# qingqing-zijin/LEAD-YOLO

Measured on AMD Instinct MI355X. Metric: images/sec (640x640) fwd+bwd, higher is better.
Workload: dtype bf16; 1 GPU; lead-yolo-s bs=64/gpu 3x640x640 bf16 full train step: uint8 batch -> train-mode forward (batch-statistics BN), ComputeLoss, HIP backward, clip 10, SGD-nesterov 3 groups, ModelEMA update (BASELINE.json configs[2]); random-init weights; global_batch=64, parallelism=dp1 (single GPU, no collective), world_size=1

## Files before the change

### lead-yolo_amd/csrc/ly_conv3x3.hip

```cpp
#include <cstdlib>
#include "ly_tile.hpp"
#include "ly_params.h"

#define LY_C3_NT 8
#define LY_C3_NV 6

#ifndef LY_C3_NTA_WPE
#define LY_C3_NTA_WPE 3
#endif
template <typename T, int MT, int WC, int NTA = 0>
__global__ __launch_bounds__(LY_THREADS) __attribute__((amdgpu_waves_per_eu(sizeof(T) == 2 ? (NTA > 0 ? LY_C3_NTA_WPE : 3) : 2))) void ly_conv3x3_kernel(const LyConv3Params P, const int gy, const int tiles_x, const int tiles_y, const int rp, const int ps) {
  using TR = LyT<T>;
  using RV = typename TR::RV;
  constexpr int VW = TR::VW, PL = TR::PL;
  constexpr int LY_CC = 8 * VW;
  constexpr int KS = LY_CC / 32;
  constexpr int LY_RSH = ly_qrs(KS);
  extern __shared__ f32x4 ly_smem4[];
  const int TH = P.TH, TW = P.TW, FW = TW + 2;
  const int frame = (TH + 2) * FW;
  char* hs_hi = reinterpret_cast<char*>(ly_smem4);
  char* hs_lo = hs_hi + (PL - 1) * 4 * ps;
  const T* const x = reinterpret_cast<const T*>(P.x);
  T* const out = reinterpret_cast<T*>(P.out);

  const int tid = threadIdx.x, lane = tid & 63;
  const int wave = __builtin_amdgcn_readfirstlane(tid >> 6);
  const int li = lane & 15, lq = lane >> 4;
  constexpr int WP = 4 / WC;
  constexpr int NTW = LY_C3_NT / WP;
  const int wc = wave % WC, wp = wave / WC;
  int b = ly_xcd_remap((int)blockIdx.x, (int)gridDim.x);
  const int by = b % gy; b /= gy;
  const int tx = b % tiles_x; b /= tiles_x;
  const int ty = b % tiles_y;
  const int n_img = b / tiles_y;
  const int h0 = ty * TH, w0 = tx * TW;
  const int npx = TH * TW;
  const int ntv = (npx + 15) >> 4;
  const f32x4 zero = ly_zero4();
  const int C32 = (P.Cin + 31) >> 5;
  const int NCH = (P.Cin + LY_CC - 1) / LY_CC;
  const int S = 9 * C32;
  const int Tt = (P.N + 15) >> 4;
  const long img0 = (long)n_img * P.H * P.W;

  int hb[NTW];
  long orow[NTW];
#pragma unroll
  for (int n = 0; n < NTW; ++n) {
    const int p = 16 * (wp * NTW + n) + li;
    const int pp = p < npx ? p : 0;
    const int r = pp / TW, c = pp - r * TW;
    hb[n] = r * rp + c * LY_RSH;
    const bool ok = p < npx && h0 + r < P.H && w0 + c < P.W;
    orow[n] = ok ? img0 + (long)(h0 + r) * P.W + (w0 + c) : -1;
  }

  const int items = frame * 8;
  int src[LY_C3_NV];
  int dst[LY_C3_NV];
#pragma unroll
  for (int e = 0; e < LY_C3_NV; ++e) {
    const int idx = tid + e * LY_THREADS;
    int off = -1;
    int dd = 0;
    if (idx < items) {
      const int pos = idx >> 3, c4 = idx & 7;
      const int fr = pos / FW, fc = pos - fr * FW;
      const int hh = h0 - 1 + fr, ww = w0 - 1 + fc;
      dd = fr * rp + fc * LY_RSH;
      if (hh >= 0 && hh < P.H && ww >= 0 && ww < P.W) off = (int)((img0 + (long)hh * P.W + ww) * P.ldx + VW * c4);
    }
    src[e] = off; dst[e] = dd;
  }
  RV pv[LY_C3_NV];
  auto prefetch = [&](int c0) {
#pragma unroll
    for (int e = 0; e < LY_C3_NV; ++e) {
      const int c4 = (tid + e * LY_THREADS) & 7;
      const bool ok = src[e] >= 0 && c0 + VW * c4 < P.Cin;
      pv[e] = ly_ldrv<T>(ok ? x + src[e] + c0 : x);
    }
  };
  auto commit = [&](int c0) {
#pragma unroll
    for (int e = 0; e < LY_C3_NV; ++e) {
      const int idx = tid + e * LY_THREADS;
      const int c4 = idx & 7;
      const bool ok = src[e] >= 0 && c0 + VW * c4 < P.Cin;
      RV v = pv[e];
      if (!ok) ly_zero_raw(v);
      if (idx < items) ly_img_put_rv(hs_hi, hs_lo, dst[e], ps, VW * c4, v);
    }
  };

  f32x4 acc[MT][NTW];
#pragma unroll
  for (int t = 0; t < MT; ++t)
#pragma unroll
    for (int n = 0; n < NTW; ++n) acc[t][n] = zero;
  long wbase[MT];
#pragma unroll
  for (int t = 0; t < MT; ++t) {
    const int tt = (by * WC + wc) * MT + t;
    wbase[t] = (long)(tt < Tt ? tt : Tt - 1) * S;
  }
  const uint4* wpk = reinterpret_cast<const uint4*>(P.wp);
  ly_l2_warm(P.wp, (long)Tt * S * PL * 1024, P.stats ? reinterpret_cast<float*>(P.stats) : reinterpret_cast<float*>(P.out));

  auto wstep = [&](int tap, int cc, int ks) -> long {
    int st = KS * cc + ks;
    if (st >= C32) st = C32 - 1;
    return (long)tap * C32 + st;
  };
  LyWF<PL> wcur[MT], wnxt[MT];
#pragma unroll
  for (int t = 0; t < MT; ++t) wcur[t] = ly_wfragp<PL>(wpk, wbase[t], lane);

  prefetch(0);
  commit(0);
  __syncthreads();

  for (int cc = 0; cc < NCH; ++cc) {
    const bool more = cc + 1 < NCH;
    prefetch((more ? cc + 1 : cc) * LY_CC);
#pragma unroll(MT * NTW <= 8 ? 1 : 9)
    for (int tap = 0; tap < 9; ++tap) {
      const int toff = (tap / 3) * rp + (tap % 3) * LY_RSH;
#pragma unroll
      for (int ks = 0; ks < KS; ++ks) {
        {
          const bool last = ks == KS - 1;
          const int nk = last ? 0 : ks + 1;
          const int nt = last ? (tap < 8 ? tap + 1 : 0) : tap;
          const int nc = (last && tap == 8) ? (more ? cc + 1 : cc) : cc;
#pragma unroll
          for (int t = 0; t < MT; ++t) wnxt[t] = ly_wfragp<PL>(wpk, wbase[t] + wstep(nt, nc, nk), lane);
        }
        if constexpr (NTA > 0) {
          bf16x8 xh[NTA], xl[NTA];
#pragma unroll
          for (int n = 0; n < NTA; ++n) {
            xh[n] = ly_img_frag(hs_hi, hb[n] + toff, ps, ks, lq);
            xl[n] = xh[n];
            if constexpr (PL == 2) xl[n] = ly_img_frag(hs_lo, hb[n] + toff, ps, ks, lq);
          }
#pragma unroll
          for (int n = 0; n < NTA; ++n)
#pragma unroll
            for (int t = 0; t < MT; ++t) acc[t][n] = ly_mfmap<PL>(wcur[t], xh[n], xl[n], acc[t][n]);
        } else {
#pragma unroll
        for (int n = 0; n < NTW; ++n) {
          if (wp * NTW + n < ntv) {
            const bf16x8 xh = ly_img_frag(hs_hi, hb[n] + toff, ps, ks, lq);
            bf16x8 xl = xh;
            if constexpr (PL == 2) xl = ly_img_frag(hs_lo, hb[n] + toff, ps, ks, lq);
#pragma unroll
            for (int t = 0; t < MT; ++t) acc[t][n] = ly_mfmap<PL>(wcur[t], xh, xl, acc[t][n]);
          }
        }
        }
#pragma unroll
        for (int t = 0; t < MT; ++t) wcur[t] = wnxt[t];
      }
    }
    if (more) {
      __syncthreads();
      commit((cc + 1) * LY_CC);
      __syncthreads();
    }
  }

  const int act = P.act;
  const bool vec_ok = (P.ldo & 3) == 0;
#pragma unroll
  for (int t = 0; t < MT; ++t) {
    const int tt = (by * WC + wc) * MT + t;
    const int c = 16 * tt + 4 * lq;
    if (tt >= Tt || c >= P.N) continue;
    float sc[4], sh[4];
#pragma unroll
    for (int r = 0; r < 4; ++r) {
      const bool ok = c + r < P.N;
      sc[r] = (ok && P.e_scale) ? P.e_scale[c + r] : 1.f;
      sh[r] = (ok && P.e_shift) ? P.e_shift[c + r] : 0.f;
    }
    f32x4 s1 = zero, s2 = zero;
#pragma unroll
    for (int n = 0; n < NTW; ++n) {
      if (orow[n] < 0) continue;
      f32x4 u;
#pragma unroll
      for (int r = 0; r < 4; ++r) u[r] = acc[t][n][r] * sc[r] + sh[r];
      if (P.stats) {
        s1 += u;
        s2 += u * u;
        if (!out) continue;
      }
      const f32x4 v = ly_act4(u, act);
      T* o = out + orow[n] * P.ldo + c;
      if (vec_ok && c + 3 < P.N) {
        ly_st4<T>(o, v);
      } else {
#pragma unroll
        for (int r = 0; r < 4; ++r)
          if (c + r < P.N) ly_st1<T>(o + r, v[r]);
      }
    }
    if (P.stats) ly_stats_flush(P.stats, P.N, c, s1, s2);
  }
}

#ifndef LY_C3_PD
#define LY_C3_PD 3
#endif
template <int V>
struct LyC3Ic { static constexpr int value = V; };

template <typename T, int MT, int WC>
__global__ __launch_bounds__(LY_THREADS) __attribute__((amdgpu_waves_per_eu(2))) void ly_conv3x3_lat_kernel(const LyConv3Params P, const int gy, const int tiles_x, const int tiles_y, const int rp, const int ps) {
  using TR = LyT<T>;
  using RV = typename TR::RV;
  constexpr int VW = TR::VW, PL = TR::PL;
  constexpr int LY_CC = 8 * VW;
  constexpr int KS = LY_CC / 32;
  constexpr int LY_RSH = ly_qrs(KS);
  extern __shared__ f32x4 ly_smem4[];
  const int TH = P.TH, TW = P.TW, FW = TW + 2;
  const int frame = (TH + 2) * FW;
  char* hs_hi = reinterpret_cast<char*>(ly_smem4);
  char* hs_lo = hs_hi + (PL - 1) * 4 * ps;
  const T* const x = reinterpret_cast<const T*>(P.x);
  T* const out = reinterpret_cast<T*>(P.out);

  const int tid = threadIdx.x, lane = tid & 63;
  const int wave = __builtin_amdgcn_readfirstlane(tid >> 6);
  const int li = lane & 15, lq = lane >> 4;
  constexpr int WP = 4 / WC;
  constexpr int NTW = LY_C3_NT / WP;
  const int wc = wave % WC, wp = wave / WC;
  int b = ly_xcd_remap((int)blockIdx.x, (int)gridDim.x);
  const int by = b % gy; b /= gy;
  const int tx = b % tiles_x; b /= tiles_x;
  const int ty = b % tiles_y;
  const int n_img = b / tiles_y;
  const int h0 = ty * TH, w0 = tx * TW;
  const int npx = TH * TW;
  const int ntv = (npx + 15) >> 4;
  const f32x4 zero = ly_zero4();
  const int C32 = (P.Cin + 31) >> 5;
  const int NCH = (P.Cin + LY_CC - 1) / LY_CC;
  const int S = 9 * C32;
  const int Tt = (P.N + 15) >> 4;
  const long img0 = (long)n_img * P.H * P.W;

  int hb[NTW];
#pragma unroll
  for (int n = 0; n < NTW; ++n) {
    const int p = 16 * (wp * NTW + n) + li;
    const int pp = p < npx ? p : 0;
    const int r = pp / TW, c = pp - r * TW;
    hb[n] = r * rp + c * LY_RSH;
  }
  auto out_row = [&](int n) -> long {
    const int p = 16 * (wp * NTW + n) + li;
    const int pp = p < npx ? p : 0;
    const int r = pp / TW, c = pp - r * TW;
    const bool ok = p < npx && h0 + r < P.H && w0 + c < P.W;
    return ok ? img0 + (long)(h0 + r) * P.W + (w0 + c) : -1;
  };

  const int items = frame * 8;
  int src[LY_C3_NV];
  int dst[LY_C3_NV];
#pragma unroll
  for (int e = 0; e < LY_C3_NV; ++e) {
    const int idx = tid + e * LY_THREADS;
    int off = -1;
    int dd = 0;
    if (idx < items) {
      const int pos = idx >> 3, c4 = idx & 7;
      const int fr = pos / FW, fc = pos - fr * FW;
      const int hh = h0 - 1 + fr, ww = w0 - 1 + fc;
      dd = fr * rp + fc * LY_RSH;
      if (hh >= 0 && hh < P.H && ww >= 0 && ww < P.W) off = (int)((img0 + (long)hh * P.W + ww) * P.ldx + VW * c4);
    }
    src[e] = off; dst[e] = dd;
  }
  RV pv[LY_C3_NV];
  auto prefetch = [&](int c0) {
#pragma unroll
    for (int e = 0; e < LY_C3_NV; ++e) {
      const int c4 = (tid + e * LY_THREADS) & 7;
      const bool ok = src[e] >= 0 && c0 + VW * c4 < P.Cin;
      pv[e] = ly_ldrv<T>(ok ? x + src[e] + c0 : x);
    }
  };
  auto commit = [&](int c0) {
#pragma unroll
    for (int e = 0; e < LY_C3_NV; ++e) {
      const int idx = tid + e * LY_THREADS;
      const int c4 = idx & 7;
      const bool ok = src[e] >= 0 && c0 + VW * c4 < P.Cin;
      RV v = pv[e];
      if (!ok) ly_zero_raw(v);
      if (idx < items) ly_img_put_rv(hs_hi, hs_lo, dst[e], ps, VW * c4, v);
    }
  };

  f32x4 acc[MT][NTW];
#pragma unroll
  for (int t = 0; t < MT; ++t)
#pragma unroll
    for (int n = 0; n < NTW; ++n) acc[t][n] = zero;
  long wbase[MT];
#pragma unroll
  for (int t = 0; t < MT; ++t) {
    const int tt = (by * WC + wc) * MT + t;
    wbase[t] = (long)(tt < Tt ? tt : Tt - 1) * S;
  }
  const uint4* wpk = reinterpret_cast<const uint4*>(P.wp);
  ly_l2_warm(P.wp, (long)Tt * S * PL * 1024, P.stats ? reinterpret_cast<float*>(P.stats) : reinterpret_cast<float*>(P.out));

  auto wstep = [&](int tap, int cc, int ks) -> long {
    int st = KS * cc + ks;
    if (st >= C32) st = C32 - 1;
    return (long)tap * C32 + st;
  };
  static_assert(PL == 1, "bf16 storage only");
  constexpr int PD = LY_C3_PD;
  constexpr int SPC = 9 * KS;
  static_assert(SPC % PD == 0, "ring depth must divide the steps of a chunk");
  LyWF<PL> wq[PD][MT];
  auto wstep_at = [&](int cc, int j, bool more) -> long {
    int c2 = cc;
    if (j >= SPC) { j -= SPC; c2 = more ? cc + 1 : cc; }
    return wstep(j / KS, c2, j % KS);
  };
  {
#pragma unroll
    for (int j = 0; j < PD - 1; ++j)
#pragma unroll
      for (int t = 0; t < MT; ++t) wq[j][t] = ly_wfragp<PL>(wpk, wbase[t] + wstep_at(0, j, NCH > 1), lane);
  }

  prefetch(0);
  commit(0);
  __syncthreads();

  auto contract = [&](auto ncC) {
    constexpr int NC = decltype(ncC)::value;
    for (int cc = 0; cc < NCH; ++cc) {
      const bool more = cc + 1 < NCH;
      prefetch((more ? cc + 1 : cc) * LY_CC);
      {
#pragma unroll
        for (int tap = 0; tap < 9; ++tap) {
          int toff = (tap / 3) * rp + (tap % 3) * LY_RSH;
          asm volatile("" : "+s"(toff));
#pragma unroll
          for (int ks = 0; ks < KS; ++ks) {
            const int j = tap * KS + ks;
            int lane_j = lane;
            asm volatile("" : "+v"(lane_j));
#pragma unroll
            for (int t = 0; t < MT; ++t) wq[(j + PD - 1) % PD][t] = ly_wfragp<PL>(wpk, wbase[t] + wstep_at(cc, j + PD - 1, more), lane_j);
#pragma unroll
            for (int n = 0; n < NC; ++n) {
              {
                const bf16x8 xh = ly_img_frag(hs_hi, hb[n] + toff, ps, ks, lq);
#pragma unroll
                for (int t = 0; t < MT; ++t) acc[t][n] = ly_mfmap<PL>(wq[j % PD][t], xh, xh, acc[t][n]);
              }
            }
            __builtin_amdgcn_sched_barrier(0);
          }
        }
      }
      if (more) {
        __syncthreads();
        commit((cc + 1) * LY_CC);
        __syncthreads();
      }
    }
  };
  {
    int nw = ntv - wp * NTW;
    nw = nw < 0 ? 0 : nw > NTW ? NTW : nw;
    switch (nw) {
      case 1: contract(LyC3Ic<1>()); break;
      case 2: contract(LyC3Ic<2>()); break;
      case 3: contract(LyC3Ic<3>()); break;
      case 4: contract(LyC3Ic<(NTW >= 4 ? 4 : NTW)>()); break;
      case 5: contract(LyC3Ic<(NTW >= 5 ? 5 : NTW)>()); break;
      case 6: contract(LyC3Ic<(NTW >= 6 ? 6 : NTW)>()); break;
      case 7: contract(LyC3Ic<(NTW >= 7 ? 7 : NTW)>()); break;
      case 8: contract(LyC3Ic<(NTW >= 8 ? 8 : NTW)>()); break;
      default: contract(LyC3Ic<0>()); break;
    }
  }

  const int act = P.act;
  const bool vec_ok = (P.ldo & 3) == 0;
#pragma unroll
  for (int t = 0; t < MT; ++t) {
    const int tt = (by * WC + wc) * MT + t;
    const int c = 16 * tt + 4 * lq;
    if (tt >= Tt || c >= P.N) continue;
    float sc[4], sh[4];
#pragma unroll
    for (int r = 0; r < 4; ++r) {
      const bool ok = c + r < P.N;
      sc[r] = (ok && P.e_scale) ? P.e_scale[c + r] : 1.f;
      sh[r] = (ok && P.e_shift) ? P.e_shift[c + r] : 0.f;
    }
    f32x4 s1 = zero, s2 = zero;
#pragma unroll
    for (int n = 0; n < NTW; ++n) {
      const long orow_n = out_row(n);
      if (orow_n < 0) continue;
      f32x4 u;
#pragma unroll
      for (int r = 0; r < 4; ++r) u[r] = acc[t][n][r] * sc[r] + sh[r];
      if (P.stats) {
        s1 += u;
        s2 += u * u;
        if (!out) continue;
      }
      const f32x4 v = ly_act4(u, act);
      T* o = out + orow_n * P.ldo + c;
      if (vec_ok && c + 3 < P.N) {
        ly_st4<T>(o, v);
      } else {
#pragma unroll
        for (int r = 0; r < 4; ++r)
          if (c + r < P.N) ly_st1<T>(o + r, v[r]);
      }
    }
    if (P.stats) ly_stats_flush(P.stats, P.N, c, s1, s2);
  }
}

static int conv3_row_pitch(int TH, int TW, int rsh) {
  const int FW = TW + 2, npx = TH * TW;
  int best = FW * rsh, best_w = 1 << 30;
  for (int rp = FW * rsh; rp < FW * rsh + 256; rp += 16) {
    int worst = 0;
    for (int n = 0; 16 * n < npx; ++n) {
      int cnt[16] = {0};
      for (int li = 0; li < 16; ++li) {
        const int p = 16 * n + li, pp = p < npx ? p : 0;
        const int c = ++cnt[(((pp / TW) * rp + (pp % TW) * rsh) >> 4) & 15];
        if (p < npx && c > worst) worst = c;
      }
    }
    if (worst < best_w) { best_w = worst; best = rp; }
    if (worst <= 1) break;
  }
  return best;
}

template <typename T, int MT, int WC, bool LAT = false, int NTA = 0>
static int launch_conv3(const LyConv3Params& P, const LyOut& out) {
  const int tiles_x = (P.W + P.TW - 1) / P.TW, tiles_y = (P.H + P.TH - 1) / P.TH;
  const int gy = (P.N + 16 * MT * WC - 1) / (16 * MT * WC);
  const long n_img = P.M / ((long)P.H * P.W);
  long nb = n_img * tiles_x * tiles_y * gy;
  LY_CHECK(nb < (1L << 31), "conv3x3: grid too large");
  const int rp = conv3_row_pitch(P.TH, P.TW, ly_qrs(8 * LyT<T>::VW / 32));
  const int ps = ly_qps((P.TH + 2) * rp);
  size_t lds = LyT<T>::PL * (size_t)4 * ps;
  if constexpr (LAT)
    return LY_EMIT(out, (ly_launch_lds<ly_conv3x3_lat_kernel<T, MT, WC>>(dim3((unsigned)nb), dim3(LY_THREADS), lds, out.st, P, gy, tiles_x, tiles_y, rp, ps)),
                   "ly_conv3x3_lat_kernel<%s, %d, %d>", ly_tname<T>(), MT, WC);
  else
    return LY_EMIT(out, (ly_launch_lds<ly_conv3x3_kernel<T, MT, WC, NTA>>(dim3((unsigned)nb), dim3(LY_THREADS), lds, out.st, P, gy, tiles_x, tiles_y, rp, ps)),
                   "ly_conv3x3_kernel<%s, %d, %d, %d>", ly_tname<T>(), MT, WC, NTA);
}

template <typename T>
static int conv3_dispatch(const LyConv3Params& P, const LyOut& out) {
#ifdef LY_DEVEL
  static int mode = -1;
  if (mode < 0) { const char* e = getenv("LY_C3_MODE"); mode = e ? atoi(e) : 0; }
#else
  constexpr int mode = 0;
#endif
  if constexpr (LyT<T>::BF) {
    const long tiles = (P.M / ((long)P.H * P.W)) * ((P.W + P.TW - 1) / P.TW) * ((P.H + P.TH - 1) / P.TH);
    const bool small = tiles * ((P.N + 127) / 128) < 2 * 256;
    if (mode == 2) return launch_conv3<T, 2, 4, true>(P, out);
    if (mode == 4 || (mode == 0 && P.N > 64 && small)) return launch_conv3<T, 2, 2, true>(P, out);
  }
  const int ntv = (P.TH * P.TW + 15) >> 4;
  if (mode == 3) return launch_conv3<T, 2, 2>(P, out);
  if (mode == 1 || P.N > 64) {
    if constexpr (LyT<T>::BF) {
      if (mode == 0 && ntv == 5) return launch_conv3<T, 2, 4, false, 5>(P, out);
      if (mode == 0 && ntv == 8) return launch_conv3<T, 2, 4, false, 8>(P, out);
    }
    return launch_conv3<T, 2, 4>(P, out);
  }
  if constexpr (LyT<T>::BF) {
    if (mode == 0 && ntv == 8) return launch_conv3<T, 2, 2, false, 4>(P, out);
  }
  return launch_conv3<T, 2, 2>(P, out);
}

static int conv3_entry(const LyConv3Params* p, const LyOut& out) {
  LY_CHECK(p, "conv3x3: null params");
  const LyConv3Params& P = *p;
  LY_CHECK(P.dtype == LY_F32 || P.dtype == LY_BF16, "conv3x3: unknown dtype %d", P.dtype);
  const int vw = P.dtype == LY_BF16 ? 8 : 4;
  LY_CHECK(P.x && P.wp && (P.out || P.stats), "conv3x3: null pointer");
  LY_CHECK(P.M > 0 && P.H > 0 && P.W > 0 && P.Cin > 0 && P.N > 0, "conv3x3: bad sizes");
  LY_CHECK((P.Cin & 3) == 0 && P.ldx % vw == 0 && P.ldx >= (P.Cin + vw - 1) / vw * vw && ((uintptr_t)P.x & 15) == 0,
           "conv3x3: Cin=%d must be a multiple of 4, ldx=%d a multiple of %d covering Cin rounded up to it", P.Cin, P.ldx, vw);
  LY_CHECK(P.M % ((long)P.H * P.W) == 0, "conv3x3: M is not a whole number of images");
  LY_CHECK(P.TH >= 1 && P.TW >= 1 && P.TH * P.TW <= 16 * LY_C3_NT, "conv3x3: patch %dx%d exceeds %d pixels", P.TH, P.TW, 16 * LY_C3_NT);
  LY_CHECK((P.TH + 2) * (P.TW + 2) * 8 <= LY_C3_NV * LY_THREADS, "conv3x3: frame of patch %dx%d exceeds the staging capacity", P.TH, P.TW);
  LY_CHECK(P.M * (long)P.ldx < (1L << 31), "conv3x3: input exceeds the 31-bit offsets of the staging plan");
  return P.dtype == LY_BF16 ? conv3_dispatch<__bf16>(P, out) : conv3_dispatch<float>(P, out);
}

extern "C" int ly_conv3x3_fwd(const LyConv3Params* p, void* stream) { return conv3_entry(p, LY_ON_STREAM(stream)); }

extern "C" int ly_conv3x3_describe(const LyConv3Params* p, char* name, int cap) {
  LY_CHECK(name && cap > 0, "conv3x3_describe: bad arguments");
  return conv3_entry(p, LyOut{nullptr, name, cap});
}
```

Baseline: 7175 images/sec.

## Replace double-buffered weight fragments with configurable-depth register ring in conv3x3

Replaces the wcur/wnxt double buffer of global weight fragments with a ring of PD register slots, so loads are issued PD-1 steps ahead of their MFMA use. The tap loop is split into unrolled tap groups so the ring indices stay compile-time constants. For the bf16 NTA==8 variant, scheduling barriers pin load issue order relative to the MFMAs. This aims to hide global/L2 weight-load latency, at the cost of more VGPRs (possible occupancy loss or spills) and a constrained compiler schedule.

Result: no change. 7174 images/sec (-0.0%).

```diff
diff --git a/lead-yolo_amd/csrc/ly_conv3x3.hip b/lead-yolo_amd/csrc/ly_conv3x3.hip
--- a/lead-yolo_amd/csrc/ly_conv3x3.hip
+++ b/lead-yolo_amd/csrc/ly_conv3x3.hip
@@ -7,6 +7,12 @@
 
 #ifndef LY_C3_NTA_WPE
 #define LY_C3_NTA_WPE 3
+#endif
+#ifndef LY_C3_PIN
+#define LY_C3_PIN(BF, WC, NTA) ((BF) && (NTA) == 8)
+#endif
+#ifndef LY_C3_TPD
+#define LY_C3_TPD(BF, WC, NTA) ((BF) ? 2 : 3)
 #endif
 template <typename T, int MT, int WC, int NTA = 0>
 __global__ __launch_bounds__(LY_THREADS) __attribute__((amdgpu_waves_per_eu(sizeof(T) == 2 ? (NTA > 0 ? LY_C3_NTA_WPE : 3) : 2))) void ly_conv3x3_kernel(const LyConv3Params P, const int gy, const int tiles_x, const int tiles_y, const int rp, const int ps) {
@@ -114,9 +120,21 @@
     if (st >= C32) st = C32 - 1;
     return (long)tap * C32 + st;
   };
-  LyWF<PL> wcur[MT], wnxt[MT];
-#pragma unroll
-  for (int t = 0; t < MT; ++t) wcur[t] = ly_wfragp<PL>(wpk, wbase[t], lane);
+  constexpr int PD = LY_C3_TPD(sizeof(T) == 2, WC, NTA);
+  constexpr bool PIN = LY_C3_PIN(sizeof(T) == 2, WC, NTA);
+  constexpr int SPC = 9 * KS;
+  constexpr int TU = MT * NTW > 8 ? 9 : 3;
+  static_assert(PD >= 2 && (TU * KS) % PD == 0, "ring depth must divide the steps of an unrolled tap group");
+  LyWF<PL> wq[PD][MT];
+  auto wstep_at = [&](int cc, int j, bool more) -> long {
+    int c2 = cc;
+    if (j >= SPC) { j -= SPC; c2 = more ? cc + 1 : cc; }
+    return wstep(j / KS, c2, j % KS);
+  };
+#pragma unroll
+  for (int j = 0; j < PD - 1; ++j)
+#pragma unroll
+    for (int t = 0; t < MT; ++t) wq[j][t] = ly_wfragp<PL>(wpk, wbase[t] + wstep_at(0, j, NCH > 1), lane);
 
   prefetch(0);
   commit(0);
@@ -125,19 +143,18 @@
   for (int cc = 0; cc < NCH; ++cc) {
     const bool more = cc + 1 < NCH;
     prefetch((more ? cc + 1 : cc) * LY_CC);
-#pragma unroll(MT * NTW <= 8 ? 1 : 9)
-    for (int tap = 0; tap < 9; ++tap) {
+#pragma unroll(MT * NTW <= 8 ? 1 : 3)
+    for (int tg = 0; tg < 9; tg += TU) {
+#pragma unroll
+    for (int td = 0; td < TU; ++td) {
+      const int tap = tg + td;
       const int toff = (tap / 3) * rp + (tap % 3) * LY_RSH;
 #pragma unroll
       for (int ks = 0; ks < KS; ++ks) {
-        {
-          const bool last = ks == KS - 1;
-          const int nk = last ? 0 : ks + 1;
-          const int nt = last ? (tap < 8 ? tap + 1 : 0) : tap;
-          const int nc = (last && tap == 8) ? (more ? cc + 1 : cc) : cc;
-#pragma unroll
-          for (int t = 0; t < MT; ++t) wnxt[t] = ly_wfragp<PL>(wpk, wbase[t] + wstep(nt, nc, nk), lane);
-        }
+        const int j = tap * KS + ks;
+#pragma unroll
+        for (int t = 0; t < MT; ++t) wq[(td * KS + ks + PD - 1) % PD][t] = ly_wfragp<PL>(wpk, wbase[t] + wstep_at(cc, j + PD - 1, more), lane);
+        if constexpr (PIN) __builtin_amdgcn_sched_barrier(0);
         if constexpr (NTA > 0) {
           bf16x8 xh[NTA], xl[NTA];
 #pragma unroll
@@ -149,7 +166,7 @@
 #pragma unroll
           for (int n = 0; n < NTA; ++n)
 #pragma unroll
-            for (int t = 0; t < MT; ++t) acc[t][n] = ly_mfmap<PL>(wcur[t], xh[n], xl[n], acc[t][n]);
+            for (int t = 0; t < MT; ++t) acc[t][n] = ly_mfmap<PL>(wq[(td * KS + ks) % PD][t], xh[n], xl[n], acc[t][n]);
         } else {
 #pragma unroll
         for (int n = 0; n < NTW; ++n) {
@@ -158,13 +175,13 @@
             bf16x8 xl = xh;
             if constexpr (PL == 2) xl = ly_img_frag(hs_lo, hb[n] + toff, ps, ks, lq);
 #pragma unroll
-            for (int t = 0; t < MT; ++t) acc[t][n] = ly_mfmap<PL>(wcur[t], xh, xl, acc[t][n]);
+            for (int t = 0; t < MT; ++t) acc[t][n] = ly_mfmap<PL>(wq[(td * KS + ks) % PD][t], xh, xl, acc[t][n]);
           }
         }
         }
-#pragma unroll
-        for (int t = 0; t < MT; ++t) wcur[t] = wnxt[t];
-      }
+        if constexpr (PIN) __builtin_amdgcn_sched_barrier(0);
+      }
+    }
     }
     if (more) {
       __syncthreads();
```
